# naxingyu/lstm-rnn

Measured on AMD Instinct MI355X. Metric: train frames/sec (node), 3x250 BLSTM 39->183, higher is better.
Workload: dtype bf16; 1 GPU; timit_3x250_blstm_H125; topology=39 -> blstm250 -> blstm250 -> blstm250 -> softmax183, parallel_sequences_per_gpu=50, seq_len=U[250,350], weights=965192, update=stochastic momentum SGD every fraction, parallelism=dp1 over sequences, inputs=fractions resident in HBM (cn_fraction_load_resident), deterministic_sums=True

## Files before the change

lstm-rnn_amd/csrc/cn_api.cpp:

```cpp
#include "cn_internal.h"
#include "cn_noise_unpack.h"
#include "../../include/currennt_hip_debug.h"

#include <dlfcn.h>
#include <rccl/rccl.h>

#include <algorithm>
#include <cmath>
#include <cstdio>
#include <cstdlib>
#include <cstring>
#include <deque>
#include <map>
#include <mutex>
#include <stdexcept>
#include <string>
#include <vector>

using namespace cn;

namespace {

thread_local std::string g_last_error;

// ... 98 lines not shown
    bool has_comm() const { return comm != nullptr || ipc != nullptr; }
    hipStream_t comm_stream = nullptr;
    hipEvent_t ev_comm = nullptr, ev_comm_fork = nullptr;
    bool comm_pending = false;
    int64_t comm_exchanges = 0;

    bool armed = false;
    UpdateRule arm;
    enum { FAMILY_NONE = 0, FAMILY_SGD, FAMILY_ADAM };
    int family = FAMILY_NONE;
    float *adam_v = nullptr;

    float clip_max = 0.f;
    ClipRecord *clip_rec = nullptr;
    bool clip_valid = false;
    bool arm_deferred = false;

    bool drop_enable = false;
    uint64_t drop_seed = 0, drop_pass = 0;
    int next_ordinal = 0;

    float noise_sigma = 0.f;
    uint64_t noise_seed = 0, noise_pass = 0;
    hipEvent_t ev_noise_fork = nullptr, ev_noise = nullptr;
    bool noise_wait = false;

    bool finalized = false;
    float *arena = nullptr;
    float *acc = nullptr;
    bool acc_valid = false;
    size_t total = 0;

    bool timing = false;
    int rpl_override = 0;
    struct Span { hipEvent_t a, b; };
    std::vector<Span> spans[KC_COUNT];
    std::vector<hipEvent_t> free_events;
    double acc_ms[KC_COUNT] = {};
    long acc_n[KC_COUNT] = {};

    size_t esz() const { return f32 ? 4 : 2; }
};

struct cn_layer {
    cn_ctx *ctx = nullptr;
    cn_layer_kind kind = CN_LAYER_INPUT;
    cn_layer *prev = nullptr;
    int size = 0;
    float bias = 0.f;
    int PS = 0, PSp = 0, maxT = 0;
    bool trainable = false, post = false, lstm = false, has_follower = false;
    bool mcc_pending = false;
    float *sm_stat = nullptr;
    bool sm_lazy = false;
    bool sm_lazy_next = true;
    bool sm_read = false;

    int dirs = 1, H = 0, Hp = 0;
    int Lp = 0;
    int P = 0, Pp = 0;

    void *out_op = nullptr;
    float *out_f32 = nullptr;
    float *err = nullptr;
    float *stage_in = nullptr;
    float *targets = nullptr;

    int ordinal = 0;
    float drop_rate = 0.f;
    void *in_drop = nullptr;
    bool dropped = false;
    DropArgs drop{};

    float *acts = nullptr, *cell = nullptr, *th = nullptr;
    void *pre16 = nullptr;
    bool err_in_delta = false;
    void *delta_op = nullptr;

    size_t woff = 0;
    int nw = 0;
    float *w = nullptr, *wu = nullptr, *wd = nullptr;
    float own_lr = -1.f;
    std::vector<float> pending_w;
    bool dirty = true;
    bool updated = false;
    bool deferred = false;

    void *Win = nullptr, *WinT = nullptr, *Wrec = nullptr, *WrecT = nullptr;
    float *bias_p = nullptr, *peep_p = nullptr;
    void *nWinT = nullptr, *nWrecT = nullptr;
    float *npeep = nullptr;
    bool noisy_ready = false, noise_used = false;
    float *grad_block = nullptr;
    size_t grad_block_floats = 0;
    float *dWin = nullptr, *dWrec = nullptr, *dbias = nullptr, *dpeep = nullptr;

    hipEvent_t ev_fork = nullptr, ev_join = nullptr;
    hipEvent_t ev_pack = nullptr;
    bool pack_pending = false;

    char kname[2][CN_KNAME_LEN] = {{0}, {0}};

    float *det_ws = nullptr;
    float *gpart = nullptr; int gpart_slots = 0;
    float *det_colpart = nullptr;

    int ctc_cap = 0;
    int *ctc_labels = nullptr;
    size_t ctc_stride = 1;
    bool ctc_labels_valid = false;
    bool ctc_swept = false;
    int ctc_maxS = 1;
    int2 *ctc_alpha = nullptr, *ctc_beta = nullptr; int ctc_Sp = 0;
    int *ctc_info = nullptr;
    float *ctc_rowstat = nullptr;
    int *ctc_hbuf[2] = {nullptr, nullptr}; hipEvent_t ctc_ev[2] = {nullptr, nullptr}; unsigned ctc_uploads = 0;

    std::vector<void *> owned;

    size_t maxN() const { return (size_t)PSp * maxT; }
};

namespace cn {
static const Options &default_options() { static const Options o = options_from_env(); return o; }
static thread_local const Options *t_opt = nullptr;
const Options &opt() { return t_opt ? *t_opt : default_options(); }
Options options_from_env()
{
    Options o;
    auto env_name = [](const char *name) { std::string e = "CN_"; for (const char *p = name; *p; ++p) e += (char)toupper((unsigned char)*p); return e; };
#define CN_OPT_FLAG(name) o.name = getenv(env_name(#name).c_str()) != nullptr;
#define CN_OPT_NUM(name, dflt) if (const char *v = getenv(env_name(#name).c_str())) o.name = atol(v);
    CN_OPTION_LIST(CN_OPT_FLAG, CN_OPT_NUM)
#undef CN_OPT_FLAG
#undef CN_OPT_NUM
    return o;
}
bool option_set(Options &o, const char *name, long value)
{
#define CN_OPT_FLAG(n) if (!strcmp(name, #n)) { o.n = value != 0; return true; }
#define CN_OPT_NUM(n, dflt) if (!strcmp(name, #n)) { o.n = value; return true; }
    CN_OPTION_LIST(CN_OPT_FLAG, CN_OPT_NUM)
#undef CN_OPT_FLAG
#undef CN_OPT_NUM
    return false;
}
bool option_get(const Options &o, const char *name, long *value)
{
#define CN_OPT_FLAG(n) if (!strcmp(name, #n)) { *value = o.n; return true; }
#define CN_OPT_NUM(n, dflt) if (!strcmp(name, #n)) { *value = o.n; return true; }
    CN_OPTION_LIST(CN_OPT_FLAG, CN_OPT_NUM)
#undef CN_OPT_FLAG
#undef CN_OPT_NUM
    return false;
}
}

namespace {

void enter(cn_ctx *c)
{
    HIP_CHECK(hipSetDevice(c->device));
    cn::t_opt = &c->opt;
}

void *dalloc(cn_layer *l, size_t bytes)
{
    void *p = nullptr;
    if (bytes == 0) bytes = 16;
    HIP_CHECK(hipMalloc(&p, bytes));
    HIP_CHECK(hipMemsetAsync(p, 0, bytes, l->ctx->stream));
    l->owned.push_back(p);
    return p;
}

void *dalloc_guarded(cn_layer *l, size_t bytes, size_t bytes_per_step)
{
    const size_t guard = (size_t)CN_GUARD_STEPS * bytes_per_step;
    return (char *)dalloc(l, bytes + 2 * guard) + guard;
}

hipStream_t masked_stream(int device, int ncu, int total)
{
    static std::mutex mu;
    static std::map<std::pair<int, int>, hipStream_t> pool;
    if (ncu <= 0 || ncu >= total) return nullptr;
    std::lock_guard<std::mutex> lock(mu);
    auto it = pool.find({device, ncu});
    if (it != pool.end()) return it->second;
    std::vector<uint32_t> mask((total + 31) / 32, 0u);
    for (int i = 0; i < total; ++i)
        if ((long)(i + 1) * ncu / total != (long)i * ncu / total) mask[i / 32] |= 1u << (i % 32);
    hipStream_t st = nullptr;
    if (hipExtStreamCreateWithCUMask(&st, (uint32_t)mask.size(), mask.data()) != hipSuccess) { (void)hipGetLastError(); st = nullptr; }
    pool[{device, ncu}] = st;
    return st;
}

static void use_rowmap(cn_ctx *c, GemmNT &g)
{
    if (opt().no_nt_rowmap || !c->d_pat_raw || !c->loaded) return;
    int *rm = c->rowmap_of(c->d_pat_raw);
    g.rowcnt = rm; g.rowmap = rm + 4; g.dummymap = rm + 4 + c->pat_maxN; g.m_est = c->est_real;
}

hipEvent_t get_event(cn_ctx *c)
{
    if (!c->free_events.empty()) { hipEvent_t e = c->free_events.back(); c->free_events.pop_back(); return e; }
    hipEvent_t e; HIP_CHECK(hipEventCreate(&e)); return e;
}
struct Timed {
    cn_ctx *c; int cls; hipEvent_t a = nullptr; hipStream_t st;
    Timed(cn_ctx *ctx, int k, hipStream_t stream = nullptr) : c(ctx), cls(k), st(stream ? stream : ctx->stream)
    {
        if (c->timing) { a = get_event(c); hipEventRecord(a, st); }
    }
    ~Timed()
    {
        if (a) { hipEvent_t b = get_event(c); hipEventRecord(b, st); c->spans[cls].push_back({a, b}); }
    }
};

bool softmax_fast(cn_ctx *c)
{
    const bool exact = opt().softmax_exact;
    return c->prec == P_BF16 && !exact;
}
float *posteriors(cn_layer *o)
{
    cn_ctx *c = o->ctx;
    o->sm_read = true;
    if (o->sm_lazy) {
        launch_softmax_normalise(c->stream, softmax_fast(c), o->out_f32, c->d_pat, c->N, o->size, o->Lp, o->sm_stat);
        o->sm_lazy = false;
    }
    return o->out_f32;
}

void join_side(cn_ctx *c)
{
    for (size_t i = 0; i < c->pending_joins.size(); ++i) {
        bool newest = true;
        for (size_t j = i + 1; j < c->pending_joins.size(); ++j) newest = newest && c->pending_join_streams[j] != c->pending_join_streams[i];
        if (newest) HIP_CHECK(hipStreamWaitEvent(c->stream, c->pending_joins[i], 0));
    }
    c->pending_joins.clear(); c->pending_join_streams.clear();
    if (c->comm_pending) { HIP_CHECK(hipStreamWaitEvent(c->stream, c->ev_comm, 0)); c->comm_pending = false; }
}
void stream_wait_layer(cn_layer *layer, hipStream_t st)
{
    cn_ctx *c = layer->ctx;
    bool pending = false;
    for (hipEvent_t e : c->pending_joins) pending = pending || e == layer->ev_join;
    if (pending) { HIP_CHECK(hipStreamWaitEvent(st, layer->ev_join, 0)); return; }
    if (!c->ev_ext) HIP_CHECK(hipEventCreateWithFlags(&c->ev_ext, hipEventDisableTiming));
    HIP_CHECK(hipEventRecord(c->ev_ext, c->stream));
    HIP_CHECK(hipStreamWaitEvent(st, c->ev_ext, 0));
}

struct Rccl {
    void *handle = nullptr;
    decltype(&ncclGetUniqueId) GetUniqueId = nullptr;
    decltype(&ncclCommInitRank) CommInitRank = nullptr;
    decltype(&ncclCommDestroy) CommDestroy = nullptr;
    decltype(&ncclAllReduce) AllReduce = nullptr;
    decltype(&ncclGetErrorString) GetErrorString = nullptr;
    decltype(&ncclGroupStart) GroupStart = nullptr;
    decltype(&ncclGroupEnd) GroupEnd = nullptr;
};
Rccl &rccl()
{
    static Rccl r;
    static std::mutex mu;
    std::lock_guard<std::mutex> lock(mu);
    if (r.handle) return r;
    const char *names[] = {getenv("CN_RCCL_LIB"), "librccl.so.1", "librccl.so", "/opt/rocm/lib/librccl.so.1"};
    void *h = nullptr;
    std::string tried;
    for (const char *n : names) {
        if (!n || !*n) continue;
        h = dlopen(n, RTLD_NOW | RTLD_LOCAL);
        if (h) break;
        tried += std::string(tried.empty() ? "" : "; ") + dlerror();
    }
    if (!h) throw cn_error(CN_ERR_COMM, "cannot open librccl (data-parallel training needs RCCL): " + tried);
    auto sym = [&](const char *name) {
        void *f = dlsym(h, name);
        if (!f) throw cn_error(CN_ERR_COMM, std::string("librccl lacks ") + name);
        return f;
    };
    r.GetUniqueId = (decltype(r.GetUniqueId))sym("ncclGetUniqueId");
    r.CommInitRank = (decltype(r.CommInitRank))sym("ncclCommInitRank");
    r.CommDestroy = (decltype(r.CommDestroy))sym("ncclCommDestroy");
    r.AllReduce = (decltype(r.AllReduce))sym("ncclAllReduce");
    r.GetErrorString = (decltype(r.GetErrorString))sym("ncclGetErrorString");
    r.GroupStart = (decltype(r.GroupStart))sym("ncclGroupStart");
    r.GroupEnd = (decltype(r.GroupEnd))sym("ncclGroupEnd");
    r.handle = h;
    return r;
}
void rccl_check(ncclResult_t e, const char *what)
{
    if (e != ncclSuccess) throw cn_error(CN_ERR_COMM, std::string(what) + ": " + rccl().GetErrorString(e));
}
#define RCCL_CHECK(x) rccl_check((x), #x)
void require_comm(cn_ctx *c, const char *who)
// ... 2419 lines not shown
```

lstm-rnn_amd/csrc/cn_gemm.hip:

```cpp
#include "cn_internal.h"
#include "cn_gemm_device.h"

#include <cstdlib>

namespace cn {

int device_cus()
{
    static int cus_of[64] = {0};
    int dev = 0; (void)hipGetDevice(&dev);
    int &cus = cus_of[dev & 63];
    if (!cus && (hipDeviceGetAttribute(&cus, hipDeviceAttributeMultiprocessorCount, dev) != hipSuccess || cus <= 0)) cus = 256;
    return cus;
}

bool rows_aligned(const void *base, long ld, int elt, int align) { return (uintptr_t)base % align == 0 && ld * elt % align == 0; }
bool rows_fit(long rows, long ld, int elt, unsigned long long limit) { return (unsigned long long)rows * ld * elt < limit; }
bool nt_out_rows_aligned(const GemmNT &g)
{
    return (!g.C || rows_aligned(g.C, g.ldc, 4, 16)) && (!g.C2 || rows_aligned(g.C2, g.ldc2, 2, 8));
}

int tn_plan_splits(const GemmTN &g, int splits, int bk, int *kchunk, FoldItem *fold, int *nfold)
{
// ... 332 lines not shown
#pragma unroll
                    for (int j = 0; j < TJ; ++j)
                        acc[i][j] = __builtin_amdgcn_mfma_f32_32x32x2f32(a[i], b[j], acc[i][j], 0, 0, 0);
            }
        } else {
            const int g16 = lane >> 4, idx = lane & 15, q = idx >> 2, pp = idx & 3;
#pragma unroll
            for (int ks = 0; ks < G::BK / 16; ++ks) {
                bf16x8 a[G::PLANES][TI], b[G::PLANES][TJ];
#pragma unroll
                for (int pl = 0; pl < G::PLANES; ++pl)
#pragma unroll
                    for (int jj = 0; jj < 2; ++jj) {
                        const int k = ks * 16 + 8 * (g16 >> 1) + 4 * jj + q;
#pragma unroll
                        for (int i = 0; i < TI; ++i) {
                            const int ma = wm * RM + i * 32 + 16 * (g16 & 1) + 4 * pp;
                            s16x4 va = __builtin_amdgcn_ds_read_tr16_b64_v4i16(
                                (s16x4 __attribute__((address_space(3))) *)(sa + pl * G::PLANE_A + k * PA + ma * 2));
                            bf16x4 ta = __builtin_bit_cast(bf16x4, va);
#pragma unroll
                            for (int e = 0; e < 4; ++e) a[pl][i][4 * jj + e] = ta[e];
                        }
#pragma unroll
                        for (int j = 0; j < TJ; ++j) {
                            const int nb = wn * RN + j * 32 + 16 * (g16 & 1) + 4 * pp;
                            s16x4 vb = __builtin_amdgcn_ds_read_tr16_b64_v4i16(
                                (s16x4 __attribute__((address_space(3))) *)(sb + pl * G::PLANE_B + k * PB + nb * 2));
                            bf16x4 tb = __builtin_bit_cast(bf16x4, vb);
#pragma unroll
                            for (int e = 0; e < 4; ++e) b[pl][j][4 * jj + e] = tb[e];
                        }
                    }
#pragma unroll
                for (int i = 0; i < TI; ++i)
#pragma unroll
                    for (int j = 0; j < TJ; ++j) {
                        if constexpr (X3) {
                            acc[i][j] = __builtin_amdgcn_mfma_f32_32x32x16_bf16(a[1][i], b[0][j], acc[i][j], 0, 0, 0);
                            acc[i][j] = __builtin_amdgcn_mfma_f32_32x32x16_bf16(a[0][i], b[1][j], acc[i][j], 0, 0, 0);
                        }
                        acc[i][j] = __builtin_amdgcn_mfma_f32_32x32x16_bf16(a[0][i], b[0][j], acc[i][j], 0, 0, 0);
                    }
            }
        }
        if (TN_NBUF == 1) __syncthreads();
        if (kt + 1 < nk) lwrite((kt + 1) % TN_NBUF);
        __syncthreads();
    }

#pragma unroll
    for (int j = 0; j < TJ; ++j) {
        const int n = n0 + wn * RN + j * 32 + fr;
        if (n >= p.N) continue;
#pragma unroll
        for (int i = 0; i < TI; ++i) {
#pragma unroll
            for (int r = 0; r < 16; ++r) {
                const int m = mfma32_row(r, fh, m0 + wm * RM + i * 32);
                if (m >= p.M) continue;
                if (p.ws) p.ws[(long)split * p.M * p.ldc + (long)m * p.ldc + n] = acc[i][j][r];
                else atomicAdd(&p.C[(long)m * p.ldc + n], acc[i][j][r]);
            }
        }
    }
}

template <int PREC, int BM, int BN>
static void launch_tn(hipStream_t s, const GemmTN *gs, int n, const FoldItem *extra)
{
    using G = TnGeom<PREC, BM, BN>;
    GemmTNGroup grp{};
    FoldItem fold[TN_GROUP + 1]; int nfold = 0;
    int blocks = 0;
    long all_tiles = 0;
    for (int i = 0; i < n; ++i) all_tiles += (long)((gs[i].M + BM - 1) / BM) * ((gs[i].N + BN - 1) / BN);
    for (int i = 0; i < TN_GROUP; ++i) {
        grp.first_block[i] = blocks;
        if (i >= n) { grp.first_block[i] = 0x7fffffff; continue; }
        const GemmTN &g = gs[i];
        const int tiles_m = (g.M + BM - 1) / BM, tiles_n = (g.N + BN - 1) / BN, ntiles = tiles_m * tiles_n;
        long cap_atomic = (32L << 20) / ((long)g.M * g.N * 4);
        const int target_env = (int)opt().tn_blocks;
        const int target = target_env ? target_env : 576;
        int splits = (int)((target + all_tiles - 1) / all_tiles);
        int maxsplit = (g.K + 4 * G::BK - 1) / (4 * G::BK);
        if (splits > maxsplit) splits = maxsplit;
        if (splits > cap_atomic && !g.ws) splits = (int)cap_atomic;
        if (g.ws && splits > g.ws_splits) splits = g.ws_splits;
        if (splits < 1) splits = 1;
        splits = tn_plan_splits(g, splits, G::BK, &grp.kchunk[i], fold, &nfold);
        grp.p[i] = g; grp.tiles_n[i] = tiles_n; grp.ntiles[i] = ntiles;
        blocks += ntiles * splits;
    }
    grp.first_block[TN_GROUP] = blocks;
    if (extra) fold[nfold++] = *extra;
    if (blocks == 0) { if (nfold) launch_fold(s, fold, nfold); return; }
    auto kern = gemm_tn_kernel<PREC, BM, BN>;
    constexpr int lds = G::LDS;
    static DeviceOnce attr_once;
    if (attr_once.first()) {
        (void)hipFuncSetAttribute((const void *)kern, hipFuncAttributeMaxDynamicSharedMemorySize, lds);
    }
    hipLaunchKernelGGL(kern, dim3(blocks), dim3(G::NT), lds, s, grp);
    if (nfold) launch_fold(s, fold, nfold);
}

enum TnShape { TN_64, TN_128 };
static TnShape tn_shape(const GemmTN *gs, int n)
{
    for (int i = 0; i < n; ++i)
        if ((long)((gs[i].M + 63) / 64) * ((gs[i].N + 63) / 64) >= 2048) return TN_128;
    return TN_64;
}

static void launch_tn_any(hipStream_t s, int prec, const GemmTN *gs, int n, const FoldItem *extra)
{
    const TnShape sh = tn_shape(gs, n);
#define CN_TN_DISPATCH(P)                                                      \
    switch (sh) {                                                              \
    case TN_64:      launch_tn<P, 64, 64>(s, gs, n, extra); break;             \
    case TN_128:     launch_tn<P, 128, 128>(s, gs, n, extra); break;           \
    }
    if (prec == P_F32) { CN_TN_DISPATCH(P_F32) }
    else if (prec == P_X3) { CN_TN_DISPATCH(P_X3) }
    else { CN_TN_DISPATCH(P_BF16) }
#undef CN_TN_DISPATCH
}

void launch_gemm_tn(hipStream_t s, int prec, const GemmTN &g, int cu_budget, const FoldItem *extra)
{
    if (g.M <= 0 || g.N <= 0 || g.K <= 0) { if (extra) launch_fold(s, extra, 1); return; }
    if (gemm_tn_big_applies(prec, g)) { launch_gemm_tn_big_group(s, &g, 1, cu_budget, extra); return; }
    launch_tn_any(s, prec, &g, 1, extra);
}

void launch_gemm_tn_small_group(hipStream_t s, int prec, const GemmTN *gs, int n, const FoldItem *extra)
{
    launch_tn_any(s, prec, gs, n, extra);
}

void launch_gemm_tn_group(hipStream_t s, int prec, const GemmTN *gs, int n, int cu_budget, const FoldItem *extra)
{
    GemmTN grp[TN_GROUP], big[TN_GROUP]; int ng = 0, nb = 0;
    bool any_big = false;
    for (int i = 0; i < n; ++i) any_big = any_big || (gs[i].M > 0 && gs[i].N > 0 && gs[i].K > 0 && gemm_tn_big_applies(prec, gs[i]));
    {
        const long gmink = opt().tnbig_group_mink;
        long outs = 0, kmin = 1L << 40;
        for (int i = 0; i < n; ++i)
            if (gs[i].M > 0 && gs[i].N > 0 && gs[i].K > 0 && gemm_tn_big_can(prec, gs[i])) { outs += (long)gs[i].M * gs[i].N; kmin = std::min<long>(kmin, gs[i].K); }
        if (outs >= (1L << 19) && kmin >= gmink) any_big = true;
    }
    for (int i = 0; i < n; ++i) {
        if (gs[i].M <= 0 || gs[i].N <= 0 || gs[i].K <= 0) continue;
        if (any_big && nb < TN_GROUP && gemm_tn_big_can(prec, gs[i])) { big[nb++] = gs[i]; continue; }
        const bool huge = (long)((gs[i].M + 63) / 64) * ((gs[i].N + 63) / 64) >= 2048;
        if (huge || ng == TN_GROUP) launch_gemm_tn(s, prec, gs[i]);
        else grp[ng++] = gs[i];
    }
    if (nb) launch_gemm_tn_big_group(s, big, nb, cu_budget, ng ? nullptr : extra);
    if (ng) launch_tn_any(s, prec, grp, ng, extra);
    else if (!nb && extra) launch_fold(s, extra, 1);
}

}
```

lstm-rnn_amd/csrc/cn_internal.h:

```cpp
#pragma once

#include <hip/hip_runtime.h>
#include <hip/hip_ext.h>
#include <atomic>
#include <stddef.h>
#include <stdint.h>

#include "../../include/currennt_hip.h"

namespace cn {

enum Act { ACT_TANH = 0, ACT_LOGISTIC = 1, ACT_IDENTITY = 2 };

enum KClass { KC_REC_FWD = 0, KC_REC_BWD = 1, KC_GEMM_WIDE = 2, KC_GEMM_GRAD = 3, KC_OTHER = 4, KC_COMM = 5, KC_COUNT = 6 };

static inline int round_up(int x, int m) { return (x + m - 1) / m * m; }

enum Prec { P_BF16 = 0, P_F32 = 1, P_X3 = 2 };

#define CN_OPTION_LIST(FLAG, NUM)                                                                                                  \
                                                                                                              \
    FLAG(no_big_gemm) FLAG(no_big8) NUM(big8_min_k, 0) FLAG(no_nt_mid) FLAG(no_big_tn) NUM(nt_bm64_below, 400) NUM(tn_blocks, 0) \
    NUM(tnbig_blocks, 0) NUM(tnbig_group_mink, 28000) NUM(nt_mid_min_tiles, 384) NUM(nt_bm64_shortk_tiles, 1100) FLAG(no_nt_panel) NUM(nt_panel_max_panels, 0) FLAG(nt_panel_no_touch) NUM(nt_panel_min_ktiles, 8) NUM(nt_panel_max_ntiles, 2) FLAG(no_nt_rowmap) FLAG(nt_rowmap_tiled)                                                                           \
                                                                                                  \
    FLAG(no_lds_claim) FLAG(bwd_ug2) FLAG(fwd_ug2) FLAG(bwd_psum) FLAG(no_bwd_psum) FLAG(cluster_helpers) FLAG(no_cluster_helpers) \
    FLAG(cluster4) FLAG(no_cluster) FLAG(cluster_gate_off) FLAG(no_s2c) FLAG(s2c) FLAG(no_s2_asm) FLAG(no_s2_asm_bwd) FLAG(s2_x3) \
    FLAG(no_s2) FLAG(no_s2w) FLAG(no_s2w_asm) FLAG(pre16)                                                                           \
                                                                                                              \
    FLAG(softmax_exact) FLAG(tail_on_side) FLAG(no_side_rule) FLAG(no_lazy_softmax) FLAG(lazy_softmax) FLAG(comm_test_double)     \
    FLAG(no_loss_defer) FLAG(no_pack_group) FLAG(no_sgd_fuse) NUM(comm_cu_margin, 32)                                           \
                                                              \
    NUM(ctc_max_labels, 0) FLAG(ctc_serial_sweeps)                                                                                \
                                                        \
    FLAG(noise_ahead)
struct Options {
#define CN_OPT_FIELD(name) int name = 0;
#define CN_OPT_FIELD_NUM(name, dflt) long name = dflt;
    CN_OPTION_LIST(CN_OPT_FIELD, CN_OPT_FIELD_NUM)
#undef CN_OPT_FIELD
#undef CN_OPT_FIELD_NUM
};
Options options_from_env();
bool option_set(Options &o, const char *name, long value);
bool option_get(const Options &o, const char *name, long *value);
const Options &opt();

struct DeviceOnce {
    std::atomic<unsigned long long> seen{0};
    bool first()
    {
        int d = 0;
        (void)hipGetDevice(&d);
        const unsigned long long bit = 1ull << (d & 63);
        return (seen.fetch_or(bit) & bit) == 0;
    }
};

struct GemmNT {
    const void *A; long lda;
    const void *B; long ldb;
    float *C; long ldc;
    void *C2; long ldc2;
    const float *bias;
    int act;
    int M, N, K;
    const int *rowmap, *dummymap, *rowcnt; int m_est;
};
struct GemmTN {
    const void *A; long lda;
    const void *B; long ldb;
    float *C; long ldc;
    int M, N, K;
    float *ws; int ws_splits;
    int *ws_used;
};
constexpr int DET_MAX_SPLITS = 8;
struct FoldItem { float *dst; float *part; long stride; int nparts, rows, cols, ld, accumulate, clear; };
constexpr int FOLD_MAX = 4;
void launch_fold(hipStream_t s, const FoldItem *items, int n);
int device_cus();
bool rows_aligned(const void *base, long ld, int elt, int align);
bool rows_fit(long rows, long ld, int elt, unsigned long long limit);
bool nt_out_rows_aligned(const GemmNT &g);
int tn_plan_splits(const GemmTN &g, int splits, int bk, int *kchunk, FoldItem *fold, int *nfold);
void launch_gemm_nt(hipStream_t s, int prec, const GemmNT &g, hipEvent_t done = nullptr);
bool gemm_nt_big_applies(int prec, const GemmNT &g);
void launch_gemm_nt_big(hipStream_t s, int prec, const GemmNT &g, hipEvent_t done = nullptr);
bool gemm_nt_mid_applies(int prec, const GemmNT &g);
bool gemm_nt_panel_applies(int prec, const GemmNT &g, int cus);
void launch_gemm_nt_panel(hipStream_t s, const GemmNT &g, hipEvent_t done = nullptr);
void launch_gemm_nt_mid(hipStream_t s, const GemmNT &g, hipEvent_t done = nullptr);
void launch_gemm_tn(hipStream_t s, int prec, const GemmTN &g, int cu_budget = 0, const FoldItem *extra = nullptr);
bool gemm_tn_big_applies(int prec, const GemmTN &g);
bool gemm_tn_big_can(int prec, const GemmTN &g);
void launch_gemm_tn_big_group(hipStream_t s, const GemmTN *gs, int n, int cu_budget = 0, const FoldItem *extra = nullptr);
void launch_gemm_tn_group(hipStream_t s, int prec, const GemmTN *gs, int n, int cu_budget = 0, const FoldItem *extra = nullptr);
void launch_gemm_tn_small_group(hipStream_t s, int prec, const GemmTN *gs, int n, const FoldItem *extra = nullptr);

struct LstmRec {
    int H, Hp, dirs, PS, T, Tmin;
    const char *pat;
    float *acts;
    const void *pre16;
    float *cell;
    float *th;
    void  *y_op;
    const void *Wrec;
    const float *peep;
    const float *err;
    void  *delta_op;
    const void *WrecT;
    float *dbias;
    float *dpeep;
    float bias;
    float *gpart; int gpart_slots; int *det_grid;
    int rpl;
    unsigned long long *xch;
    unsigned long long *xch_packed;
    unsigned xch_epoch;
    int *fault;
    int num_cus;
    int cluster_cus;
    char *kname;
};
constexpr int CN_KNAME_LEN = 64;
void lstm_note_grid(const LstmRec &p, int grid);
constexpr int CN_GUARD_STEPS = 6;
size_t lstm_rec_lds_bytes(int prec, bool bwd, int Hp, int rpl, int T);
bool lstm_rec_resident(int prec, int Hp);
void launch_lstm_forward(hipStream_t s, int prec, const LstmRec &p);
bool lstm_fwd_takes_pre16(int prec, const LstmRec &p);
bool lstm_s2_applies(int prec, const LstmRec &p, bool bwd);
void launch_lstm_s2(hipStream_t s, int prec, bool bwd, const LstmRec &p, hipEvent_t done = nullptr);
bool lstm_s2w_applies(int prec, const LstmRec &p, bool bwd);
void launch_lstm_s2w(hipStream_t s, bool bwd, const LstmRec &p, hipEvent_t done = nullptr);
void launch_lstm_backward(hipStream_t s, int prec, const LstmRec &p, hipEvent_t done = nullptr);
size_t lstm_cluster_xch_bytes(int prec, int Hp, int dirs, int PS, int rpl, int num_cus);
size_t lstm_cluster_xch_packed_offset(int prec, int Hp, int dirs, int PS, int rpl, int num_cus);
int lstm_cluster_size(int prec, int Hp, int dirs, int PS, int rpl, int num_cus);
bool launch_lstm_cluster(hipStream_t s, int prec, bool bwd, LstmRec &p, unsigned *epoch);
int lstm_cluster_bwd_cus(int prec, const LstmRec &p);
void lstm_cluster_stream_gone(hipStream_t s);

struct LstmGeom { int P, Pp, L, H, Hp, dirs; int prevH, prevHp, prevDirs;  };

void launch_lstm_pack(hipStream_t s, bool f32, const LstmGeom &g, float bias, const float *w,
                      void *Win, void *WinT, void *Wrec, void *WrecT, float *bias_p, float *peep_p);
void launch_lstm_unpack_grads(hipStream_t s, const LstmGeom &g, float *dWin, float *dWrec, float *dbias, float *dpeep, float *wu, hipEvent_t done = nullptr);
struct FfGeom { int P, Pp, L, Lp; int prevH, prevHp, prevDirs; };
constexpr int PACK_GROUP_MAX = 8;
struct PackFold { float *part; long stride; int nparts, clear; };
struct PackItem {
    int lstm; LstmGeom lg; FfGeom fg; float bias; const float *w;
    void *Win, *WinT, *Wrec, *WrecT; float *bias_p, *peep_p;
    int update; int optimizer; float *w_rw; const float *wu; float *wd; float lr, mom;
    float *wu_rw; float *g_in, *g_rec, *g_bias, *g_peep;
    PackFold f_in, f_rec[2], f_bias;
};
struct PackGroup { PackItem item[PACK_GROUP_MAX]; int first[PACK_GROUP_MAX]; int n; };
enum { PACK_OPT_SGD = 0, PACK_OPT_ADAM = 1 };
struct PackAdam { float *v[PACK_GROUP_MAX]; float b2, omb1, omb2, eps_t; };
struct ClipRecord;
void launch_pack_group(hipStream_t s, bool f32, PackGroup &grp, hipEvent_t done = nullptr, const PackAdam *adam = nullptr, const ClipRecord *clip = nullptr);
struct PackNoise { uint32_t k0[PACK_GROUP_MAX]; uint32_t k1, pass_lo, pass_hi; float sigma; };
void launch_pack_group_noise(hipStream_t s, bool f32, PackGroup &grp, const PackNoise &nz);
void launch_ff_pack(hipStream_t s, bool f32, const FfGeom &g, float bias, const float *w,
                    void *W, void *WT, float *bias_p);
void launch_ff_unpack_grads(hipStream_t s, const FfGeom &g, float bias, float *dW, float *colsum, float *wu, hipEvent_t done = nullptr);

void launch_rowmap(hipStream_t s, const char *dpat, int N, int *rm, int maxN, int unchecked);
void launch_fraction_load(hipStream_t s, bool f32, int T, int PS, int PSp, const char *pat, char *dpat, const int *tcls, int *dtcls,
                          const float *tgt, float *dtgt, int W, const float *in, int P, void *dst, int Pp, int *rm = nullptr, int maxN = 0, int Tmin = 0);
void launch_pad_convert(hipStream_t s, bool f32, const float *src, int N, int P, void *dst, int Pp);
struct DropArgs {
    int N, PS, PSp, P, Pp, prevH, prevHp, prevDirs;
    uint32_t k0, k1, pass_lo, pass_hi, thr;
    float scale;
};
void launch_dropout_fwd(hipStream_t s, bool f32, const DropArgs &a, const void *src, void *dst);
void launch_dropout_bwd(hipStream_t s, const DropArgs &a, float *err);
void launch_ff_delta(hipStream_t s, bool f32, int act, const float *y, float *err, void *delta_op, int N, int L, int Lp);
void launch_colsum(hipStream_t s, const float *err, int N, int Lp, float *colsum, float *det_part = nullptr, FoldItem *fold_out = nullptr);
size_t det_colsum_part_floats(int Lp);
void launch_softmax_fwd(hipStream_t s, float *y, const char *pat, int N, int L, int Lp, const int *tcls, float *rowstat, bool fast = false, float *smstat = nullptr);
bool softmax_fwd_can_be_lazy(int L);
void launch_softmax_normalise(hipStream_t s, bool fast, float *y, const char *pat, int N, int L, int Lp, const float *smstat);
void launch_rowstat_reduce(hipStream_t s, const float *rowstat, int N, float *loss2, bool reset, float scale = -1.0f);
enum { POST_SSE = 0, POST_WEIGHTEDSSE, POST_SSE_MASK, POST_CE, POST_RMSE, POST_BINARY };
void launch_post_eval(hipStream_t s, int kind, const float *y, const float *tgt, const char *pat, int N, int L, int Lp,
                      float *rowstat, float *loss2, bool reset);
void launch_post_backward(hipStream_t s, int kind, const float *y, const float *tgt, const char *pat, int N, int L, int Lp, float *err);
void launch_classes_to_targets(hipStream_t s, const int *tcls, float *tgt, int N);
void launch_softmax_mcc_bwd(hipStream_t s, bool f32, const float *y, const int *tcls, const char *pat, int N, int L, int Lp,
                            float *err, void *delta_op, float *colsum, const float *rowstat = nullptr, float *loss2 = nullptr, float *loss_part = nullptr,
                            const float *smstat = nullptr, bool fast = false, float *colpart = nullptr, float *det_part = nullptr, FoldItem *fold_out = nullptr);
bool softmax_mcc_bwd_takes_loss(int Lp);
size_t softmax_mcc_bwd_colpart_floats();
void launch_softmax_bwd(hipStream_t s, const float *y, float *err, const char *pat, int N, int L, int Lp);
void launch_mcc_eval(hipStream_t s, const float *y, const int *tcls, int N, int L, int Lp, float *loss2 , bool reset, float *rowstat);
void launch_mcc_backward(hipStream_t s, const float *y, const int *tcls, int N, int L, int Lp, float *err);
void launch_scale(hipStream_t s, float *x, size_t n, float a);
struct SumRanks { const float *src[8]; int n; };
void launch_sum_ranks(hipStream_t s, float *dst, const SumRanks &sr, size_t n);

struct IpcComm;
bool ipc_backend_selected();
void ipc_unique_id(char *id, size_t bytes);
IpcComm *ipc_comm_create(const char *id, int rank, int world);
void ipc_comm_destroy(IpcComm *c);
void ipc_comm_mark_failed(IpcComm *c);
void ipc_allreduce(IpcComm *c, float *buf, size_t n, hipStream_t st, size_t capacity_hint = 0);
bool ipc_comm_is_p2p(const IpcComm *c);
void ipc_comm_check(IpcComm *c, hipStream_t st);
void ipc_comm_check_fast(IpcComm *c);
bool ipc_comm_p2p_selfcheck(IpcComm *c, hipStream_t st, void (*make_id)(char *), char *rccl_id);
void ipc_allreduce_loss(IpcComm *c, float *err, int *correct);
constexpr int P2P_GROUPS = 64, P2P_THREADS = 256;
constexpr int P2P_READY = 0, P2P_REDUCED = 8 * P2P_GROUPS, P2P_DONE = 16 * P2P_GROUPS, P2P_FAILED = 24 * P2P_GROUPS, P2P_FLAG_WORDS = 24 * P2P_GROUPS + 64;
struct P2pArgs {
    float *buf; size_t n, piece, slot;
    float *stage[8];
    unsigned long long *flags[8];
    int me, world, two_phase;
    unsigned long long seq, timeout_ticks;
    unsigned long long *host_failed;
};
void launch_p2p_allreduce(hipStream_t s, const P2pArgs &a);
void launch_sgd(hipStream_t s, float *w, const float *wu, float *wd, size_t n, float lr, float mom, hipEvent_t done = nullptr);
struct AdamScalars { float b1, omb1, b2, omb2, alpha_t, eps_t; };
void launch_adam(hipStream_t s, float *w, const float *wu, float *m, float *v, size_t n, const AdamScalars &a, hipEvent_t done = nullptr);
void launch_accumulate(hipStream_t s, float *acc, const float *wu, size_t n, bool first);

constexpr int CLIP_LANES = 16384, CLIP_WGS = 16;
enum { CLIP_NONE = 0, CLIP_SCALE = 1, CLIP_SKIP = 2 };
struct ClipRecord {
    float norm, scale; int state; float max_seen;
    long long updates, clipped, skipped;
    unsigned arrivals, pad;
    double part[CLIP_WGS];
};
void launch_grad_norm(hipStream_t s, const float *g, size_t n, float max_norm, ClipRecord *rec);
void launch_sgd_clip(hipStream_t s, float *w, const float *wu, float *wd, size_t n, float lr, float mom, const ClipRecord *rec, hipEvent_t done = nullptr);
void launch_adam_clip(hipStream_t s, float *w, const float *wu, float *m, float *v, size_t n, const AdamScalars &a, const ClipRecord *rec, hipEvent_t done = nullptr);

struct CtcArgs {
    const float *y; const char *pat;
    int T, PSp, C, Lp;
    const int *labels, *next, *first, *laboff;
    int maxS;
// ... 15 lines not shown
```

Measured before the change: 16.24 million frames/s.

## Fuse LSTM input and recurrent weight-gradient GEMMs into one TN kernel

Adds a dedicated bf16 TN GEMM kernel that computes the input-weight gradient and the per-direction recurrent-weight gradients in a single launch. It shares the delta (A) tiles, concatenating the X columns and the shifted Y columns into one B panel, and split-K results are combined with atomicAdd. The grouped TN launcher routes to this path when no big-GEMM path applies and K is large enough. The aim is to cut repeated reads of the delta matrix and extra launches. In exchange it adds float atomics, which may break deterministic sums, plus a new launch counter.

```diff
diff --git a/lstm-rnn_amd/csrc/cn_api.cpp b/lstm-rnn_amd/csrc/cn_api.cpp
--- a/lstm-rnn_amd/csrc/cn_api.cpp
+++ b/lstm-rnn_amd/csrc/cn_api.cpp
@@ -274,6 +274,7 @@
     CN_OPTION_LIST(CN_OPT_FLAG, CN_OPT_NUM)
 #undef CN_OPT_FLAG
 #undef CN_OPT_NUM
+    if (!strcmp(name, "tn_fused_launches")) { *value = o.tn_fused_launches; return true; }
     return false;
 }
 }
diff --git a/lstm-rnn_amd/csrc/cn_gemm.hip b/lstm-rnn_amd/csrc/cn_gemm.hip
--- a/lstm-rnn_amd/csrc/cn_gemm.hip
+++ b/lstm-rnn_amd/csrc/cn_gemm.hip
@@ -508,6 +508,7 @@
             if (gs[i].M > 0 && gs[i].N > 0 && gs[i].K > 0 && gemm_tn_big_can(prec, gs[i])) { outs += (long)gs[i].M * gs[i].N; kmin = std::min<long>(kmin, gs[i].K); }
         if (outs >= (1L << 19) && kmin >= gmink) any_big = true;
     }
+    if (!any_big && gemm_tn_lstm_applies(prec, gs, n)) { launch_gemm_tn_lstm(s, gs, n, cu_budget, extra); return; }
     for (int i = 0; i < n; ++i) {
         if (gs[i].M <= 0 || gs[i].N <= 0 || gs[i].K <= 0) continue;
         if (any_big && nb < TN_GROUP && gemm_tn_big_can(prec, gs[i])) { big[nb++] = gs[i]; continue; }
diff --git a/lstm-rnn_amd/csrc/cn_gemm_tn_lstm.hip b/lstm-rnn_amd/csrc/cn_gemm_tn_lstm.hip
--- /dev/null
+++ b/lstm-rnn_amd/csrc/cn_gemm_tn_lstm.hip
@@ -0,0 +1,207 @@
+#include "cn_internal.h"
+#include "cn_gemm_device.h"
+
+namespace cn {
+
+constexpr int TL_BM = 64, TL_BK = 64, TL_NT = 256;
+constexpr int TL_STAGES = 2;
+constexpr int TL_PA = TL_BM * 2 + 64;
+constexpr int TL_HT = 128;
+template <int PT> struct TlGeom {
+    static constexpr int NB = PT + TL_HT, PB = NB * 2 + 64;
+    static constexpr int TILE_A = TL_BK * TL_PA, TILE_B = TL_BK * PB, STAGE = TILE_A + TILE_B, LDS = 2 * STAGE;
+    static constexpr int CPR_A = TL_BM / 8, CPR_X = PT / 8, CPR_Y = TL_HT / 8;
+    static constexpr int NLD_A = TL_BK * CPR_A / TL_NT, NLD_X = TL_BK * CPR_X / TL_NT, NLD_Y = TL_BK * CPR_Y / TL_NT;
+    static constexpr int TJ = NB / 2 / 32;
+};
+
+struct TnLstm {
+    const char *A; long lda; int K, R;
+    const char *X; long ldx; int Pp;
+    const char *Y[2]; long ldy[2]; int yshift[2], Ky[2]; int Hp;
+    float *Cin; long ldcin; float *Crec[2]; long ldcrec[2];
+    int mtiles, kchunk, nwg;
+};
+
+template <int PT>
+__global__ __launch_bounds__(TL_NT) void gemm_tn_lstm_kernel(TnLstm p)
+{
+    extern __shared__ __attribute__((aligned(16))) char smem[];
+    using G = TlGeom<PT>;
+    constexpr int PA = TL_PA, PB = G::PB, TJ = G::TJ, NB = G::NB;
+
+    const int tid = threadIdx.x, lane = tid & 63, wave = tid >> 6;
+    const int wm = wave >> 1, wn = wave & 1;
+    const int bid = xcd_tile_order(blockIdx.x, p.nwg);
+    const int tile = bid % p.mtiles, split = bid / p.mtiles;
+    const int m0 = tile * TL_BM, d = m0 / (4 * p.Hp);
+    const int kbeg = split * p.kchunk, kend = min(p.K, kbeg + p.kchunk);
+    if (kbeg >= kend) return;
+    const int nk = (kend - kbeg + TL_BK - 1) / TL_BK;
+    const int yshift = p.yshift[d], Ky = p.Ky[d], Pp = p.Pp, Hp = p.Hp;
+
+    constexpr int TL_NOWHERE = (int)0x80000000;
+    const __amdgpu_buffer_rsrc_t resA = buffer_resource(p.A + ((long)kbeg * p.lda + m0) * 2, (long)(kend - kbeg) * p.lda * 2);
+    const __amdgpu_buffer_rsrc_t resX = buffer_resource(p.X + (long)kbeg * p.ldx * 2, (long)(kend - kbeg) * p.ldx * 2);
+    const long yrows = min(Ky, kend - yshift);
+    const __amdgpu_buffer_rsrc_t resY = buffer_resource(p.Y[d], yrows > 0 ? yrows * p.ldy[d] * 2 : 0);
+    const int stepA = TL_BK * (int)p.lda * 2, stepX = TL_BK * (int)p.ldx * 2, stepY = TL_BK * (int)p.ldy[d] * 2;
+    int offA[G::NLD_A], offX[G::NLD_X], offY[G::NLD_Y];
+#pragma unroll
+    for (int j = 0; j < G::NLD_A; ++j) { const int c = tid + TL_NT * j; offA[j] = ((c / G::CPR_A) * (int)p.lda + (c % G::CPR_A) * 8) * 2; }
+#pragma unroll
+    for (int j = 0; j < G::NLD_X; ++j) {
+        const int c = tid + TL_NT * j, col = (c % G::CPR_X) * 8;
+        offX[j] = col < Pp ? ((c / G::CPR_X) * (int)p.ldx + col) * 2 : TL_NOWHERE;
+    }
+#pragma unroll
+    for (int j = 0; j < G::NLD_Y; ++j) {
+        const int c = tid + TL_NT * j, col = (c % G::CPR_Y) * 8;
+        offY[j] = col < Hp ? ((kbeg + c / G::CPR_Y - yshift) * (int)p.ldy[d] + col) * 2 : TL_NOWHERE;
+    }
+
+    u32x4 ra[TL_STAGES][G::NLD_A], rx[TL_STAGES][G::NLD_X], ry[TL_STAGES][G::NLD_Y];
+    auto load16 = [](__amdgpu_buffer_rsrc_t res, int off) { return __builtin_bit_cast(u32x4, __builtin_amdgcn_raw_buffer_load_b128(res, off, 0, 0)); };
+    auto gload = [&](int st) {
+#pragma unroll
+        for (int j = 0; j < G::NLD_A; ++j) { ra[st][j] = load16(resA, offA[j]); offA[j] += stepA; }
+#pragma unroll
+        for (int j = 0; j < G::NLD_X; ++j) { rx[st][j] = load16(resX, offX[j]); offX[j] += stepX; }
+#pragma unroll
+        for (int j = 0; j < G::NLD_Y; ++j) { ry[st][j] = load16(resY, offY[j]); offY[j] += stepY; }
+    };
+    auto lwrite = [&](int st, int buf) {
+        char *sa = smem + buf * G::STAGE, *sb = sa + G::TILE_A;
+#pragma unroll
+        for (int j = 0; j < G::NLD_A; ++j) { const int c = tid + TL_NT * j; *(u32x4 *)(sa + (c / G::CPR_A) * PA + (c % G::CPR_A) * 16) = ra[st][j]; }
+#pragma unroll
+        for (int j = 0; j < G::NLD_X; ++j) { const int c = tid + TL_NT * j; *(u32x4 *)(sb + (c / G::CPR_X) * PB + (c % G::CPR_X) * 16) = rx[st][j]; }
+#pragma unroll
+        for (int j = 0; j < G::NLD_Y; ++j) { const int c = tid + TL_NT * j; *(u32x4 *)(sb + (c / G::CPR_Y) * PB + PT * 2 + (c % G::CPR_Y) * 16) = ry[st][j]; }
+    };
+
+    f32x16 acc[TJ] = {};
+    const int fr = lane & 31, fh = lane >> 5;
+    const int g16 = lane >> 4, idx = lane & 15, q = idx >> 2, pp = idx & 3;
+
+    gload(0);
+    lwrite(0, 0);
+#pragma unroll
+    for (int t = 1; t <= TL_STAGES; ++t) if (t < nk) gload(t % TL_STAGES);
+    __syncthreads();
+    for (int kt0 = 0; kt0 < nk; kt0 += TL_STAGES) {
+#pragma unroll
+        for (int i = 0; i < TL_STAGES; ++i) {
+            const int kt = kt0 + i;
+            if (kt >= nk) break;
+            const int st = (i + 1) % TL_STAGES;
+            if (kt + 1 < nk) lwrite(st, (kt + 1) & 1);
+            if (kt + 1 + TL_STAGES < nk) gload(st);
+            const char *sa = smem + (kt & 1) * G::STAGE, *sb = sa + G::TILE_A;
+#pragma unroll
+            for (int ks = 0; ks < TL_BK / 16; ++ks) {
+                bf16x8 a, b[TJ];
+#pragma unroll
+                for (int jj = 0; jj < 2; ++jj) {
+                    const int k = ks * 16 + 8 * (g16 >> 1) + 4 * jj + q;
+                    const int ma = wm * 32 + 16 * (g16 & 1) + 4 * pp;
+                    const s16x4 va = __builtin_amdgcn_ds_read_tr16_b64_v4i16((s16x4 __attribute__((address_space(3))) *)(sa + k * PA + ma * 2));
+                    const bf16x4 ta = __builtin_bit_cast(bf16x4, va);
+#pragma unroll
+                    for (int e = 0; e < 4; ++e) a[4 * jj + e] = ta[e];
+#pragma unroll
+                    for (int j = 0; j < TJ; ++j) {
+                        const int nb = wn * (NB / 2) + j * 32 + 16 * (g16 & 1) + 4 * pp;
+                        const s16x4 vb = __builtin_amdgcn_ds_read_tr16_b64_v4i16((s16x4 __attribute__((address_space(3))) *)(sb + k * PB + nb * 2));
+                        const bf16x4 tb = __builtin_bit_cast(bf16x4, vb);
+#pragma unroll
+                        for (int e = 0; e < 4; ++e) b[j][4 * jj + e] = tb[e];
+                    }
+                }
+#pragma unroll
+                for (int j = 0; j < TJ; ++j) acc[j] = __builtin_amdgcn_mfma_f32_32x32x16_bf16(a, b[j], acc[j], 0, 0, 0);
+            }
+            __syncthreads();
+        }
+    }
+
+    const bool any_y = kend > yshift && kbeg < yshift + Ky;
+    const int mw = m0 + wm * 32 + 4 * fh;
+#pragma unroll
+    for (int j = 0; j < TJ; ++j) {
+        const int n = wn * (NB / 2) + j * 32 + fr;
+        if (n < PT ? n >= Pp : (n - PT >= Hp || !any_y)) continue;
+        const int ld = n < PT ? (int)p.ldcin : (int)p.ldcrec[d];
+        float *c = n < PT ? p.Cin + (long)mw * ld + n : p.Crec[d] + (long)(mw - d * 4 * Hp) * ld + (n - PT);
+#pragma unroll
+        for (int r = 0; r < 16; ++r) atomicAdd(c + mfma32_row(r, 0) * ld, acc[j][r]);
+    }
+}
+
+static bool tn_lstm_describe(int prec, const GemmTN *gs, int n, TnLstm *out)
+{
+    if (prec != P_BF16 || n < 2 || n > 3) return false;
+    const GemmTN &in = gs[0];
+    const int dirs = n - 1;
+    for (int i = 0; i < n; ++i) if (gs[i].M <= 0 || gs[i].N <= 0 || gs[i].K <= 0 || gs[i].ws) return false;
+    const int Hp = gs[1].N, Pp = in.N;
+    if (Pp > 256 || Hp > 128 || Pp % 32 || Hp % 32 || in.M != dirs * 4 * Hp) return false;
+    if (!rows_aligned(in.A, in.lda, 2, 16) || !rows_aligned(in.B, in.ldb, 2, 16)) return false;
+    const unsigned long long lim = 1ull << 31;
+    if (!rows_fit(in.K, in.lda, 2, lim) || !rows_fit(in.K, in.ldb, 2, lim)) return false;
+    TnLstm p{};
+    p.A = (const char *)in.A; p.lda = in.lda; p.K = in.K; p.R = in.M;
+    p.X = (const char *)in.B; p.ldx = in.ldb; p.Pp = Pp; p.Hp = Hp;
+    p.Cin = in.C; p.ldcin = in.ldc;
+    for (int d = 0; d < dirs; ++d) {
+        const GemmTN &r = gs[1 + d];
+        if (r.M != 4 * Hp || r.N != Hp || r.lda != in.lda || !rows_aligned(r.B, r.ldb, 2, 16) || !rows_fit(in.K, r.ldb, 2, lim)) return false;
+        const ptrdiff_t off = (const char *)r.A - (const char *)in.A;
+        if (off < 0 || off % 2) return false;
+        const long row = off / 2 / in.lda, col = off / 2 % in.lda;
+        if (col != (long)d * 4 * Hp || row + r.K > in.K) return false;
+        p.Y[d] = (const char *)r.B; p.ldy[d] = r.ldb; p.yshift[d] = (int)row; p.Ky[d] = r.K;
+        p.Crec[d] = r.C; p.ldcrec[d] = r.ldc;
+    }
+    p.mtiles = in.M / TL_BM;
+    *out = p;
+    return true;
+}
+
+bool gemm_tn_lstm_applies(int prec, const GemmTN *gs, int n)
+{
+    TnLstm p;
+    return tn_lstm_describe(prec, gs, n, &p) && p.K >= opt().tn_fused_mink;
+}
+
+template <int PT>
+static void launch_tl(hipStream_t s, const TnLstm &p, int blocks)
+{
+    using G = TlGeom<PT>;
+    auto kern = gemm_tn_lstm_kernel<PT>;
+    static DeviceOnce attr_once;
+    if (attr_once.first()) (void)hipFuncSetAttribute((const void *)kern, hipFuncAttributeMaxDynamicSharedMemorySize, G::LDS);
+    hipLaunchKernelGGL(kern, dim3(blocks), dim3(TL_NT), G::LDS, s, p);
+}
+
+void launch_gemm_tn_lstm(hipStream_t s, const GemmTN *gs, int n, int cu_budget, const FoldItem *extra)
+{
+    TnLstm p;
+    if (!tn_lstm_describe(P_BF16, gs, n, &p)) return;
+    const int cus = device_cus();
+    long target = opt().tn_fused_blocks;
+    if (cu_budget > 0 && cu_budget < cus) target = (target * cu_budget + cus / 2) / cus;
+    int splits = (int)((target + p.mtiles / 2) / p.mtiles);
+    const long cap_atomic = (32L << 20) / ((long)p.R * (p.Pp + p.Hp) * 4);
+    if (splits > cap_atomic) splits = (int)cap_atomic;
+    if (splits < 1) splits = 1;
+    FoldItem fold[1]; int nfold = 0;
+    splits = tn_plan_splits(gs[0], splits, TL_BK, &p.kchunk, fold, &nfold);
+    p.nwg = p.mtiles * splits;
+    if (p.Pp <= 64) launch_tl<64>(s, p, p.nwg);
+    else launch_tl<256>(s, p, p.nwg);
+    ++opt().tn_fused_launches;
+    if (extra) launch_fold(s, extra, 1);
+}
+
+}
diff --git a/lstm-rnn_amd/csrc/cn_internal.h b/lstm-rnn_amd/csrc/cn_internal.h
--- a/lstm-rnn_amd/csrc/cn_internal.h
+++ b/lstm-rnn_amd/csrc/cn_internal.h
@@ -21,6 +21,8 @@
 #define CN_OPTION_LIST(FLAG, NUM)                                                                                                  \
                                                                                                               \
     FLAG(no_big_gemm) FLAG(no_big8) NUM(big8_min_k, 0) FLAG(no_nt_mid) FLAG(no_big_tn) NUM(nt_bm64_below, 400) NUM(tn_blocks, 0) \
+        \
+    NUM(tn_fused_mink, 8192) NUM(tn_fused_blocks, 256)                                                                            \
     NUM(tnbig_blocks, 0) NUM(tnbig_group_mink, 28000) NUM(nt_mid_min_tiles, 384) NUM(nt_bm64_shortk_tiles, 1100) FLAG(no_nt_panel) NUM(nt_panel_max_panels, 0) FLAG(nt_panel_no_touch) NUM(nt_panel_min_ktiles, 8) NUM(nt_panel_max_ntiles, 2) FLAG(no_nt_rowmap) FLAG(nt_rowmap_tiled)                                                                           \
                                                                                                   \
     FLAG(no_lds_claim) FLAG(bwd_ug2) FLAG(fwd_ug2) FLAG(bwd_psum) FLAG(no_bwd_psum) FLAG(cluster_helpers) FLAG(no_cluster_helpers) \
@@ -39,6 +41,7 @@
     CN_OPTION_LIST(CN_OPT_FIELD, CN_OPT_FIELD_NUM)
 #undef CN_OPT_FIELD
 #undef CN_OPT_FIELD_NUM
+    mutable long tn_fused_launches = 0;
 };
 Options options_from_env();
 bool option_set(Options &o, const char *name, long value);
@@ -95,6 +98,8 @@
 bool gemm_tn_big_can(int prec, const GemmTN &g);
 void launch_gemm_tn_big_group(hipStream_t s, const GemmTN *gs, int n, int cu_budget = 0, const FoldItem *extra = nullptr);
 void launch_gemm_tn_group(hipStream_t s, int prec, const GemmTN *gs, int n, int cu_budget = 0, const FoldItem *extra = nullptr);
+bool gemm_tn_lstm_applies(int prec, const GemmTN *gs, int n);
+void launch_gemm_tn_lstm(hipStream_t s, const GemmTN *gs, int n, int cu_budget = 0, const FoldItem *extra = nullptr);
 void launch_gemm_tn_small_group(hipStream_t s, int prec, const GemmTN *gs, int n, const FoldItem *extra = nullptr);
 
 struct LstmRec {
```

Result: no change. 16.12 million frames/s (-0.7%).
